# psmyth94/mamba-clip

Measured on AMD Instinct MI355X. Metric: image-text pairs/sec (whole node) + selective_scan HBM GB/s, higher is better.
Workload: dtype bf16; 1 GPU; C2: ViT-B/16 image + Mamba-130M text, contrastive train step (fwd+bwd+AdamW), amp_bf16; model=vit_b16-mamba130m, global_batch=256, per_gpu_batch=256, seq_len=77, image_size=224, input=resident, step_launch=eager, parallelism=dp1, library_gemm_selection=tunableop-file

## Files before the change

mamba-clip_amd/csrc/scan_bwd_pair.hip:

```cpp
#include "scan_common.h"

namespace mc {
namespace scan {

constexpr int kQW = 4;
constexpr int kQCh = 32;
constexpr int kQN = 16;
constexpr int kQP = 4;
constexpr int kQT = 8;
constexpr int kQSub = kS / kQT;
static_assert(kS == 32 && kQSub == 4 && kFineS == kQT, "the pair backward walks the forward's 32-position chunks "
              "in 8-position sub-tiles (the fine saved-state interval)");

struct BwdPairArgs {
  int batch, dim, seqlen, n_groups, n_states, nblk, total_blocks;
  int state_ratio;
  int64_t u_bs, u_ds, dt_bs, dt_ds, z_bs, z_ds, go_bs, go_ds;
  int64_t du_bs, du_ds, ddt_bs, ddt_ds, dz_bs, dz_ds;
  int64_t B_bs, B_gs, B_ns, C_bs, C_gs, C_ns;
  const void* u; const void* delta; const void* z; const void* dout;
  const void* B; const void* C;
  const float* A; const float* D; const float* delta_bias; const float* chunk_states;
  void* du; void* ddelta; void* dz;
  float* slab_bc;
  float* slab_a;
  float* slab_d;
  float* slab_bias;
};

template <int kCtrl>
__device__ __forceinline__ float qperm(float v) {
  return __int_as_float(__builtin_amdgcn_update_dpp(0, __float_as_int(v), kCtrl, 0xF, 0xF, true));
}
constexpr int kQpEven = 0xA0;
constexpr int kQpOdd = 0xF5;
constexpr int kQpXor1 = 0xB1;
constexpr int kQpXor2 = 0x4E;

__device__ __forceinline__ float halve_bit3(float a, float b) {
  float r;
  asm volatile("s_nop 1\n\t"
               "v_add_f32_dpp %0, %1, %1 row_ror:8 row_mask:0xf bank_mask:0x3\n\t"
               "v_add_f32_dpp %0, %2, %2 row_ror:8 row_mask:0xf bank_mask:0xc"
               : "=&v"(r) : "v"(a), "v"(b));
  return r;
}
__device__ __forceinline__ float halve_bit2(float a, float b) {
  float r;
  asm volatile("s_nop 1\n\t"
               "v_add_f32_dpp %0, %1, %1 row_shl:4 row_mask:0xf bank_mask:0x5\n\t"
               "v_add_f32_dpp %0, %2, %2 row_shr:4 row_mask:0xf bank_mask:0xa"
               : "=&v"(r) : "v"(a), "v"(b));
  return r;
}

__device__ __forceinline__ float pair_finish(f32x2 a, f32x2 b, int h) {
  float sa, sb, r;
  asm("v_add_f32_e32 %0, %1, %2" : "=v"(sa) : "v"(a.x), "v"(a.y));
  asm("v_add_f32_e32 %0, %1, %2" : "=v"(sb) : "v"(b.x), "v"(b.y));
  const float keep = h ? sb : sa, send = h ? sa : sb;
  asm("s_nop 1\n\t"
      "v_add_f32_dpp %0, %1, %2 quad_perm:[1,0,3,2] row_mask:0xf bank_mask:0xf bound_ctrl:1"
      : "=v"(r) : "v"(send), "v"(keep));
  return r;
}

__device__ __forceinline__ float pair_reduce16(f32x2 (&v)[8], int lane) {
  asm volatile("s_nop 1" : "+v"(v[0]), "+v"(v[1]), "+v"(v[2]), "+v"(v[3]), "+v"(v[4]), "+v"(v[5]), "+v"(v[6]),
               "+v"(v[7]));
#pragma unroll
  for (int t = 0; t < 4; ++t) {
    auto rx = __builtin_amdgcn_permlane32_swap(__float_as_uint(v[t].x), __float_as_uint(v[t + 4].x), false, false);
    auto ry = __builtin_amdgcn_permlane32_swap(__float_as_uint(v[t].y), __float_as_uint(v[t + 4].y), false, false);
    v[t] = f32x2{__uint_as_float(rx[0]), __uint_as_float(ry[0])} + f32x2{__uint_as_float(rx[1]), __uint_as_float(ry[1])};
  }
#pragma unroll
  for (int t = 0; t < 2; ++t) {
    auto rx = __builtin_amdgcn_permlane16_swap(__float_as_uint(v[t].x), __float_as_uint(v[t + 2].x), false, false);
    auto ry = __builtin_amdgcn_permlane16_swap(__float_as_uint(v[t].y), __float_as_uint(v[t + 2].y), false, false);
    v[t] = f32x2{__uint_as_float(rx[0]), __uint_as_float(ry[0])} + f32x2{__uint_as_float(rx[1]), __uint_as_float(ry[1])};
  }
  const float x = halve_bit3(v[0].x, v[1].x), y = halve_bit3(v[0].y, v[1].y);
  const float r = halve_bit2(x, y);
  return r + qperm<kQpXor2>(r);
}

__device__ __forceinline__ void glds16_asm(const void* gsrc, uint32_t m0v) {
  uint32_t keep;
  asm volatile("s_mov_b32 %0, m0\n\ts_mov_b32 m0, %2\n\ts_nop 0\n\tglobal_load_lds_dwordx4 %1, off\n\ts_mov_b32 m0, %0"
               : "=&s"(keep) : "v"(gsrc), "s"(m0v) : "memory");
}

template <typename TI>
__device__ __forceinline__ uint2 buf_ld8(__amdgpu_buffer_rsrc_t r, uint32_t off) {
  return __builtin_bit_cast(uint2, __builtin_amdgcn_raw_buffer_load_b64(r, off, 0, 0));
}
__device__ __forceinline__ void buf_st8(__amdgpu_buffer_rsrc_t r, uint32_t off, uint2 v) {
  typedef unsigned u32x2_t __attribute__((ext_vector_type(2)));
  __builtin_amdgcn_raw_buffer_store_b64(__builtin_bit_cast(u32x2_t, v), r, off, 0, 0);
}
template <typename TI>
__device__ __forceinline__ f32x2 elem2(uint2 w, int i) {
  const uint4 q = make_uint4(w.x, w.y, 0u, 0u);
  return f32x2{elem_f<TI>(q, 2 * i), elem_f<TI>(q, 2 * i + 1)};
}

template <typename TI, bool kSP, bool kZ, bool kFine>
__global__ __launch_bounds__(64 * kQW, 2) void scan_bwd_pair_kernel(const BwdPairArgs a) {
  using TW = TI;
  constexpr int kWV = 16 / (int)sizeof(TW);
  constexpr int kWL = 8 / kWV;
  constexpr int kDbcW = kS * 2 * kQN;
  extern __shared__ __attribute__((aligned(16))) char smem[];
  const int tid = threadIdx.x;
  const int lane = tid & 63;
  const int wave = __builtin_amdgcn_readfirstlane(tid >> 6);
  f32x4* bcq = reinterpret_cast<f32x4*>(smem) + wave * (kS * 2 * kQP);
  float* dbc_base = reinterpret_cast<float*>(smem + (size_t)kQW * kS * 2 * kQP * 16);
  f32x4* xst = reinterpret_cast<f32x4*>(dbc_base + 2 * kQW * kDbcW) + wave * ((kQSub - 1) * 2 * 64);

  const int lin = xcd_remap(blockIdx.x, a.total_blocks);
  const int wblk = lin % a.nblk;
  const int bg = lin / a.nblk;
  const int g = bg % a.n_groups, b = bg / a.n_groups;
  const int H = a.dim / a.n_groups;
  const int row0 = wblk * (kQCh * kQW) + wave * kQCh;
  const int nrows = max(0, min(kQCh, H - row0));
  const int ch = lane >> 1, h = lane & 1;
  const bool my_ok = ch < nrows;
  const int my_r = max(0, min(ch, nrows - 1));
  const int dbase = g * H + min(row0, H - 1);
  const int my_dc = dbase + my_r;
  const int L_ = a.seqlen;
  constexpr bool hasZ = kZ;

  auto rows_rsrc = [&](const void* base, int64_t bs, int64_t ds) __attribute__((always_inline)) {
    return make_rsrc(reinterpret_cast<const TI*>(base) + (int64_t)b * bs + (int64_t)dbase * ds,
                     nrows > 0 ? (uint32_t)(((int64_t)(nrows - 1) * ds + L_) * (int64_t)sizeof(TI)) : 0u);
  };
  const __amdgpu_buffer_rsrc_t rs_u = rows_rsrc(a.u, a.u_bs, a.u_ds);
  const __amdgpu_buffer_rsrc_t rs_d = rows_rsrc(a.delta, a.dt_bs, a.dt_ds);
  const __amdgpu_buffer_rsrc_t rs_z = rows_rsrc(hasZ ? a.z : a.u, hasZ ? a.z_bs : a.u_bs, hasZ ? a.z_ds : a.u_ds);
  const __amdgpu_buffer_rsrc_t rs_g = rows_rsrc(a.dout, a.go_bs, a.go_ds);
  const __amdgpu_buffer_rsrc_t rs_du = rows_rsrc(a.du, a.du_bs, a.du_ds);
  const __amdgpu_buffer_rsrc_t rs_dd = rows_rsrc(a.ddelta, a.ddt_bs, a.ddt_ds);
  const __amdgpu_buffer_rsrc_t rs_dz = rows_rsrc(hasZ ? a.dz : a.du, hasZ ? a.dz_bs : a.du_bs, hasZ ? a.dz_ds : a.du_ds);
  const uint32_t ro_u = (uint32_t)(my_r * a.u_ds), ro_d = (uint32_t)(my_r * a.dt_ds);
  const uint32_t ro_z = (uint32_t)(my_r * (hasZ ? a.z_ds : a.u_ds)), ro_g = (uint32_t)(my_r * a.go_ds);
  const uint32_t ro_du = (uint32_t)(my_r * a.du_ds), ro_dd = (uint32_t)(my_r * a.ddt_ds);
  const uint32_t ro_dz = (uint32_t)(my_r * (hasZ ? a.dz_ds : a.du_ds));
  const uint32_t st_mask = my_ok ? 0u : 0x80000000u;

  const __amdgpu_buffer_rsrc_t rs_B = make_rsrc(reinterpret_cast<const TW*>(a.B) + (int64_t)b * a.B_bs + (int64_t)g * a.B_gs,
                                                (uint32_t)((15 * a.B_ns + L_) * (int64_t)sizeof(TW)));
  const __amdgpu_buffer_rsrc_t rs_C = make_rsrc(reinterpret_cast<const TW*>(a.C) + (int64_t)b * a.C_bs + (int64_t)g * a.C_gs,
                                                (uint32_t)((15 * a.C_ns + L_) * (int64_t)sizeof(TW)));
  const uint32_t bo_B = (uint32_t)(((lane >> 2) * a.B_ns + 8 * (lane & 3)) * (int64_t)sizeof(TW));
  const uint32_t bo_C = (uint32_t)(((lane >> 2) * a.C_ns + 8 * (lane & 3)) * (int64_t)sizeof(TW));
  const uint32_t cs_rs = kFine ? (uint32_t)kQN : (uint32_t)(a.n_states * kQN);
  const uint32_t cs_ks = kFine ? (uint32_t)(a.dim * kQN) : (uint32_t)kQN;
  const __amdgpu_buffer_rsrc_t rs_cs =
      make_rsrc(a.chunk_states + (int64_t)b * a.dim * a.n_states * kQN + (int64_t)dbase * cs_rs,
                nrows > 0 ? ((uint32_t)(nrows - 1) * cs_rs + (uint32_t)(a.n_states - 1) * cs_ks + kQN) * 4u : 0u);

  f32x2 A2[kQP], hcar[kQP], dA2[kQP];
#pragma unroll
  for (int p = 0; p < kQP; ++p) {
    const float* ap = a.A + (int64_t)my_dc * kQN + 8 * h + 2 * p;
    A2[p] = f32x2{ap[0], ap[1]} * kLog2e;
    hcar[p] = f32x2{0.f, 0.f};
    dA2[p] = f32x2{0.f, 0.f};
  }
  const float Dv = a.D ? a.D[my_dc] : 0.f;
  const float biasv = a.delta_bias ? a.delta_bias[my_dc] : 0.f;
  float dDacc = 0.f, dbacc = 0.f;

  uint4 pB[kWL], pC[kWL];
  f32x4 px[2];
  auto load_chunk = [&](int c) __attribute__((always_inline)) {
    const uint32_t lo = c >= 0 ? (uint32_t)(c * kS) * (uint32_t)sizeof(TW) : 0x80000000u;
#pragma unroll
    for (int k = 0; k < kWL; ++k) {
      pB[k] = buf_ld16(rs_B, (bo_B + lo) + (uint32_t)(k * 16));
      pC[k] = buf_ld16(rs_C, (bo_C + lo) + (uint32_t)(k * 16));
    }
    const uint32_t ox = c > 0 ? ((uint32_t)my_r * cs_rs + (uint32_t)(c * (kFine ? kS / kQT : 1) - 1) * cs_ks + 8 * h) * 4u
                              : 0x80000000u;
    px[0] = __builtin_bit_cast(f32x4, buf_ld16(rs_cs, ox));
    px[1] = __builtin_bit_cast(f32x4, buf_ld16(rs_cs, ox + 16));
  };
  uint2 nu, nd, nz, ng;
  auto load_raw = [&](int pos) __attribute__((always_inline)) {
    const uint32_t e = (uint32_t)(pos + 4 * h);
    nu = buf_ld8<TI>(rs_u, (ro_u + e) * 2u);
    nd = buf_ld8<TI>(rs_d, (ro_d + e) * 2u);
    ng = buf_ld8<TI>(rs_g, (ro_g + e) * 2u);
    if constexpr (hasZ) {
      nz = buf_ld8<TI>(rs_z, (ro_z + e) * 2u);
    }
  };

  struct Sc {
    f32x2 dt[4], dtu[4], gy[4];
    f32x2 own_dt[2], own_gy[2];
  };
  auto scalars = [&](uint2 ru, uint2 rd, uint2 rz, uint2 rg, bool want_gy, Sc& sc) __attribute__((always_inline)) {
    f32x2 odt[2], odtu[2], ogy[2];
#pragma unroll
    for (int i = 0; i < 2; ++i) {
      const f32x2 r = elem2<TI>(rd, i) + biasv;
      const f32x2 dt = kSP ? softplus2_log1p(r) : r;
      odt[i] = dt;
      odtu[i] = my_ok ? dt * elem2<TI>(ru, i) : f32x2{0.f, 0.f};
      if (want_gy) {
        const f32x2 go = elem2<TI>(rg, i);
        const f32x2 gy = hasZ ? go * silu2(elem2<TI>(rz, i)) : go;
        ogy[i] = my_ok ? gy : f32x2{0.f, 0.f};
      }
    }
#pragma unroll
    for (int i = 0; i < 2; ++i) {
      sc.dt[i] = f32x2{qperm<kQpEven>(odt[i].x), qperm<kQpEven>(odt[i].y)};
      sc.dt[2 + i] = f32x2{qperm<kQpOdd>(odt[i].x), qperm<kQpOdd>(odt[i].y)};
      sc.dtu[i] = f32x2{qperm<kQpEven>(odtu[i].x), qperm<kQpEven>(odtu[i].y)};
      sc.dtu[2 + i] = f32x2{qperm<kQpOdd>(odtu[i].x), qperm<kQpOdd>(odtu[i].y)};
      if (want_gy) {
        sc.gy[i] = f32x2{qperm<kQpEven>(ogy[i].x), qperm<kQpEven>(ogy[i].y)};
        sc.gy[2 + i] = f32x2{qperm<kQpOdd>(ogy[i].x), qperm<kQpOdd>(ogy[i].y)};
        sc.own_gy[i] = ogy[i];
      }
      sc.own_dt[i] = odt[i];
    }
  };
  auto bpair = [&](int t, int p) __attribute__((always_inline)) -> f32x2 {
    return reinterpret_cast<const f32x2*>(bcq + t * (2 * kQP) + h * kQP + p)[0];
  };
  auto bquad = [&](int t, int p) __attribute__((always_inline)) -> f32x4 { return bcq[t * (2 * kQP) + h * kQP + p]; };

  const int nch = (L_ + kS - 1) / kS;
  constexpr bool fine = kFine;
  typedef __attribute__((address_space(3))) char lds_char_t;
  const uint32_t xst_lds = __builtin_amdgcn_readfirstlane((uint32_t)(uintptr_t)(lds_char_t*)(reinterpret_cast<char*>(xst)));
  const float* cs_lane = a.chunk_states + (int64_t)b * a.dim * a.n_states * kQN + (int64_t)(dbase + my_r) * kQN + 8 * h;
  auto issue_fine = [&](int c) __attribute__((always_inline)) {
#pragma unroll
    for (int s = 0; s < kQSub - 1; ++s) {
      const float* src = cs_lane + (int64_t)min(c * (kS / kQT) + s, a.n_states - 1) * cs_ks;
      glds16_asm(src, xst_lds + (uint32_t)(2 * s) * 1024u);
      glds16_asm(src + 4, xst_lds + (uint32_t)(2 * s + 1) * 1024u);
    }
  };
  if (fine) {
    issue_fine(nch - 1);
    __builtin_amdgcn_s_waitcnt(0x0F70);
  }
  load_chunk(nch - 1);
  load_raw((nch - 1) * kS + (fine ? kQT * (min(kQSub, (L_ - (nch - 1) * kS) / kQT) - 1) : 0));
  int buf = 0;
  for (int c = nch - 1; c >= 0; --c) {
    const int l0 = c * kS;
    const int nsub = min(kQSub, (L_ - l0) / kQT);
    float* dbc = dbc_base + (buf * kQW + wave) * kDbcW;

    {
      const int n = lane >> 2, q = lane & 3;
      float* dst = reinterpret_cast<float*>(bcq) + ((n >> 3) * kQP + ((n & 7) >> 1)) * 4 + (n & 1);
#pragma unroll
      for (int k = 0; k < kWL; ++k)
#pragma unroll
        for (int e = 0; e < kWV; ++e) {
          const int t = 8 * q + k * kWV + e;
          dst[t * (2 * kQP * 4)] = elem_f<TW>(pB[k], e);
          dst[t * (2 * kQP * 4) + 2] = elem_f<TW>(pC[k], e);
        }
    }
    f32x2 x0[kQP];
    x0[0] = px[0].lo; x0[1] = px[0].hi; x0[2] = px[1].lo; x0[3] = px[1].hi;
    if (!my_ok) {
#pragma unroll
      for (int p = 0; p < kQP; ++p) x0[p] = f32x2{0.f, 0.f};
    }
    if (fine) __builtin_amdgcn_s_waitcnt(0x0F70);
    load_chunk(c - 1);
    wave_lds_sync();

    if constexpr (fine) {
    } else {
      f32x2 x[kQP];
#pragma unroll
      for (int p = 0; p < kQP; ++p) x[p] = x0[p];
#pragma unroll 1
      for (int s = 0; s + 1 < nsub; ++s) {
        const uint2 ru = nu, rd = nd, rz = nz, rg = ng;
        load_raw(l0 + kQT * (s + 1));
        Sc sc;
        scalars(ru, rd, rz, rg, false, sc);
#pragma unroll
        for (int t = 0; t < kQT; ++t) {
#pragma unroll
          for (int p = 0; p < kQP; ++p) {
            const f32x2 arg = (t & 1) ? pk_mul_bcast<1>(A2[p], sc.dt[t >> 1]) : pk_mul_bcast<0>(A2[p], sc.dt[t >> 1]);
            const f32x2 aa = f32x2{fast_exp2(arg.x), fast_exp2(arg.y)};
            const f32x2 bb = bpair(kQT * s + t, p);
            const f32x2 bu = (t & 1) ? pk_mul_bcast<1>(bb, sc.dtu[t >> 1]) : pk_mul_bcast<0>(bb, sc.dtu[t >> 1]);
            x[p] = aa * x[p] + bu;
          }
        }
        xst[(2 * s) * 64 + lane] = f32x4{x[0].x, x[0].y, x[1].x, x[1].y};
        xst[(2 * s + 1) * 64 + lane] = f32x4{x[2].x, x[2].y, x[3].x, x[3].y};
      }
    }
    wave_lds_sync();

#pragma unroll 1
    for (int s = nsub - 1; s >= 0; --s) {
      const uint2 ru = nu, rd = nd, rz = nz, rg = ng;
      load_raw(s > 0 ? l0 + kQT * (s - 1) : (fine ? l0 - kQT : l0 - kS));
      Sc sc;
      scalars(ru, rd, rz, rg, true, sc);
      f32x4 xi01, xi23;
      {
        const int sl = s > 0 ? s - 1 : 0;
        const f32x4 l01 = xst[(2 * sl) * 64 + lane], l23 = xst[(2 * sl + 1) * 64 + lane];
        xi01 = s > 0 ? l01 : f32x4{x0[0].x, x0[0].y, x0[1].x, x0[1].y};
        xi23 = s > 0 ? l23 : f32x4{x0[2].x, x0[2].y, x0[3].x, x0[3].y};
      }
      f32x2 S2[kQT], Q2[kQT];
      f32x2 Y2[kQT];
#pragma unroll
      for (int t = 0; t < kQT; ++t) Y2[t] = f32x2{0.f, 0.f};
#pragma unroll
      for (int t = 0; t < kQT; ++t) S2[t] = Q2[t] = f32x2{0.f, 0.f};

#pragma unroll
      for (int p = 0; p < kQP; ++p) {
        __builtin_amdgcn_sched_barrier(0);
        f32x2 a2p = A2[p];
        asm volatile("" : "+v"(a2p));
        const f32x2 xin = p == 0 ? xi01.lo : (p == 1 ? xi01.hi : (p == 2 ? xi23.lo : xi23.hi));
        f32x2 as[kQT], xs[kQT];
#pragma unroll
        for (int t = 0; t < kQT; ++t) {
          const f32x2 arg = (t & 1) ? pk_mul_bcast<1>(a2p, sc.dt[t >> 1]) : pk_mul_bcast<0>(a2p, sc.dt[t >> 1]);
          as[t] = f32x2{fast_exp2(arg.x), fast_exp2(arg.y)};
        }
        {
          f32x2 x = xin;
#pragma unroll
          for (int t = 0; t < kQT; ++t) {
            const f32x2 bb = bpair(kQT * s + t, p);
            const f32x2 bu = (t & 1) ? pk_mul_bcast<1>(bb, sc.dtu[t >> 1]) : pk_mul_bcast<0>(bb, sc.dtu[t >> 1]);
            x = as[t] * x + bu;
            xs[t] = x;
          }
        }
        {
          f32x2 red[kQT];
#pragma unroll
          for (int t = 0; t < kQT; ++t)
            red[t] = (t & 1) ? pk_mul_bcast<1>(xs[t], sc.gy[t >> 1]) : pk_mul_bcast<0>(xs[t], sc.gy[t >> 1]);
          const float v = pair_reduce16(red, lane);
          if ((lane & 2) == 0)
            dbc[((kQT * s + (lane >> 3)) * 2 + 1) * kQN + 8 * h + 2 * p + ((lane >> 2) & 1)] = v;
        }
        __builtin_amdgcn_sched_barrier(0);
        {
          f32x2 lam, dap = dA2[p], ha;
          f32x2 red[kQT];
          f32x4 qn = bquad(kQT * s + kQT - 1, p);
#pragma unroll
          for (int t = kQT - 1; t >= 0; --t) {
            const f32x4 q = qn;
            if (t > 0) qn = bquad(kQT * s + t - 1, p);
            lam = (t & 1) ? pk_fma_bcast<1>(q.hi, sc.gy[t >> 1], t == kQT - 1 ? hcar[p] : ha)
                          : pk_fma_bcast<0>(q.hi, sc.gy[t >> 1], t == kQT - 1 ? hcar[p] : ha);
            if (hasZ) Y2[t] = q.hi * xs[t] + Y2[t];
            S2[t] = lam * q.lo + S2[t];
            red[t] = (t & 1) ? pk_mul_bcast<1>(lam, sc.dtu[t >> 1]) : pk_mul_bcast<0>(lam, sc.dtu[t >> 1]);
            ha = lam * as[t];
            const f32x2 hax = ha * (t > 0 ? xs[t - 1] : xin);
            Q2[t] = hax * a2p + Q2[t];
            dap = (t & 1) ? pk_fma_bcast<1>(hax, sc.dt[t >> 1], dap) : pk_fma_bcast<0>(hax, sc.dt[t >> 1], dap);
          }
          asm volatile("" : "+v"(ha), "+v"(dap));
#pragma unroll
          for (int t = 0; t < kQT; ++t) asm volatile("" : "+v"(S2[t]), "+v"(Q2[t]));
#pragma unroll
          for (int t = 0; t < kQT; ++t) asm volatile("" : "+v"(Y2[t]));
          hcar[p] = ha;
          dA2[p] = dap;
          const float v = pair_reduce16(red, lane);
          if ((lane & 2) == 0)
            dbc[((kQT * s + (lane >> 3)) * 2 + 0) * kQN + 8 * h + 2 * p + ((lane >> 2) & 1)] = v;
        }
      }
      __builtin_amdgcn_sched_barrier(0);

      float fS[4], fQ[4];
#pragma unroll
      for (int e = 0; e < 4; ++e) {
        fS[e] = pair_finish(S2[e], S2[4 + e], h);
        fQ[e] = pair_finish(Q2[e], Q2[4 + e], h) * kLn2;
      }
      float fY[4];
#pragma unroll
      for (int e = 0; e < 4; ++e) fY[e] = pair_finish(Y2[e], Y2[4 + e], h);
      float o_du[4], o_dd[4], o_dz[4];
#pragma unroll
      for (int i = 0; i < 2; ++i) {
        const f32x2 uu = elem2<TI>(ru, i);
        const f32x2 rr = elem2<TI>(rd, i) + biasv;
        const f32x2 dt = sc.own_dt[i], gy = sc.own_gy[i];
        const f32x2 S = f32x2{fS[2 * i], fS[2 * i + 1]}, Q = f32x2{fQ[2 * i], fQ[2 * i + 1]};
        f32x2 sg = f32x2{1.f, 1.f};
        if (kSP) {
          const f32x2 ep = f32x2{fast_exp2(-rr.x * kLog2e), fast_exp2(-rr.y * kLog2e)} + 1.f;
          sg = f32x2{rr.x > 20.f ? 1.f : fast_rcp(ep.x), rr.y > 20.f ? 1.f : fast_rcp(ep.y)};
        }
        const f32x2 du = Dv * gy + dt * S;
        const f32x2 dd = (uu * S + Q) * sg;
        o_du[2 * i] = du.x; o_du[2 * i + 1] = du.y;
        o_dd[2 * i] = dd.x; o_dd[2 * i + 1] = dd.y;
        if (hasZ) {
          const f32x2 zz = elem2<TI>(rz, i), go = elem2<TI>(rg, i);
          const f32x2 ez = f32x2{fast_exp2(-zz.x * kLog2e), fast_exp2(-zz.y * kLog2e)} + 1.f;
          const f32x2 sz = f32x2{fast_rcp(ez.x), fast_rcp(ez.y)};
          const f32x2 gz = go * sz * (1.f + zz * (1.f - sz));
          const f32x2 dz = gz * (Dv * uu + f32x2{fY[2 * i], fY[2 * i + 1]});
          o_dz[2 * i] = dz.x; o_dz[2 * i + 1] = dz.y;
        }
        if (my_ok) {
          const f32x2 gu = gy * uu;
          dDacc += gu.x + gu.y;
          dbacc += dd.x + dd.y;
        }
      }
      const uint32_t e0 = (uint32_t)(l0 + kQT * s + 4 * h);
      buf_st8(rs_du, ((ro_du + e0) * 2u) | st_mask, make_uint2(cvt_pk2<TI>(o_du[0], o_du[1]), cvt_pk2<TI>(o_du[2], o_du[3])));
      buf_st8(rs_dd, ((ro_dd + e0) * 2u) | st_mask, make_uint2(cvt_pk2<TI>(o_dd[0], o_dd[1]), cvt_pk2<TI>(o_dd[2], o_dd[3])));
      if (hasZ)
        buf_st8(rs_dz, ((ro_dz + e0) * 2u) | st_mask, make_uint2(cvt_pk2<TI>(o_dz[0], o_dz[1]), cvt_pk2<TI>(o_dz[2], o_dz[3])));
    }

    if (fine && c > 0) issue_fine(c - 1);
    lds_barrier();
    {
      float* slab = a.slab_bc + (((int64_t)bg * a.nblk + wblk) * L_ + l0) * (2 * kQN);
      const float* src = dbc_base + buf * kQW * kDbcW;
      for (int f = tid; f < kDbcW / 4; f += 64 * kQW) {
        f32x4 acc = reinterpret_cast<const f32x4*>(src)[f];
#pragma unroll
        for (int w = 1; w < kQW; ++w) acc += reinterpret_cast<const f32x4*>(src + w * kDbcW)[f];
        if (4 * f < (L_ - l0) * 2 * kQN) reinterpret_cast<f32x4*>(slab)[f] = acc;
      }
    }
    buf ^= 1;
  }

  if (my_ok) {
#pragma unroll
    for (int p = 0; p < kQP; ++p) {
      const int n0 = 8 * h + 2 * p;
      a.slab_a[((int64_t)b * kQN + n0) * a.dim + my_dc] = dA2[p].x;
      a.slab_a[((int64_t)b * kQN + n0 + 1) * a.dim + my_dc] = dA2[p].y;
    }
  }
  const float dD2 = dDacc + qperm<kQpXor1>(dDacc), db2 = dbacc + qperm<kQpXor1>(dbacc);
  if (my_ok && h == 0) {
    a.slab_d[(int64_t)b * a.dim + my_dc] = dD2;
    a.slab_bias[(int64_t)b * a.dim + my_dc] = db2;
  }
}

size_t bwd_pair_lds_bytes() {
  return (size_t)kQW * kS * 2 * kQP * 16 + (size_t)2 * kQW * kS * 2 * kQN * 4 + (size_t)kQW * (kQSub - 1) * 2 * 64 * 16;
}
int bwd_pair_nblk(int H) { return (H + kQCh * kQW - 1) / (kQCh * kQW); }

bool bwd_pair_ok(const mc_scan_bwd_params* p) {
  const int ib = p->itype == MC_DTYPE_F32 ? 4 : 2;
  const int wb = p->wtype == MC_DTYPE_F32 ? 4 : 2;
  if (ib != 2 || p->wtype != p->itype || p->dstate != kQN || p->seqlen % 8 || p->reverse_groups || p->u_groups)
    return false;
  auto rows = [&](const void* t, int64_t bs, int64_t ds) {
    return !t || (aligned16(t) && bs % 8 == 0 && ds % 8 == 0 &&
                  ((int64_t)(kQCh * kQW - 1) * (ds < 0 ? -ds : ds) + p->seqlen) * 2 < ((int64_t)1 << 31));
  };
  auto bc = [&](const void* t, int64_t bs, int64_t gs, int64_t ns) {
    const int64_t v = 16 / wb;
    return aligned16(t) && bs % v == 0 && gs % v == 0 && ns % v == 0 && ns >= 0 &&
           (15 * ns + p->seqlen) * wb < ((int64_t)1 << 31);
  };
  return rows(p->u, p->u_batch_stride, p->u_dim_stride) &&
         rows(p->delta, p->delta_batch_stride, p->delta_dim_stride) &&
         rows(p->z, p->z_batch_stride, p->z_dim_stride) && rows(p->dout, p->dout_batch_stride, p->dout_dim_stride) &&
         rows(p->du, p->du_batch_stride, p->du_dim_stride) &&
         rows(p->ddelta, p->ddelta_batch_stride, p->ddelta_dim_stride) &&
         rows(p->dz, p->dz_batch_stride, p->dz_dim_stride) &&
         bc(p->B, p->B_batch_stride, p->B_group_stride, p->B_dstate_stride) &&
         bc(p->C, p->C_batch_stride, p->C_group_stride, p->C_dstate_stride) &&
         (int64_t)kQCh * kQW * mc_scan_n_states(p->seqlen, p->state_interval) * kQN * 4 < ((int64_t)1 << 31);
}

template <typename TI>
static void launch_pair_t(const BwdPairArgs& a, bool sp, bool zy, hipStream_t s) {
  const size_t lds = bwd_pair_lds_bytes();
  const dim3 grid(a.total_blocks), block(64 * kQW);
  if (a.state_ratio != 1) {
    if (sp && zy) hipLaunchKernelGGL((scan_bwd_pair_kernel<TI, true, true, true>), grid, block, lds, s, a);
    else if (sp) hipLaunchKernelGGL((scan_bwd_pair_kernel<TI, true, false, true>), grid, block, lds, s, a);
    else if (zy) hipLaunchKernelGGL((scan_bwd_pair_kernel<TI, false, true, true>), grid, block, lds, s, a);
    else hipLaunchKernelGGL((scan_bwd_pair_kernel<TI, false, false, true>), grid, block, lds, s, a);
    return;
  }
  if (sp && zy) hipLaunchKernelGGL((scan_bwd_pair_kernel<TI, true, true, false>), grid, block, lds, s, a);
  else if (sp) hipLaunchKernelGGL((scan_bwd_pair_kernel<TI, true, false, false>), grid, block, lds, s, a);
  else if (zy) hipLaunchKernelGGL((scan_bwd_pair_kernel<TI, false, true, false>), grid, block, lds, s, a);
  else hipLaunchKernelGGL((scan_bwd_pair_kernel<TI, false, false, false>), grid, block, lds, s, a);
}

void launch_bwd_pair(const mc_scan_bwd_params* p, float* slab_bc, float* slab_a, float* slab_d, float* slab_bias,
                     int nblk, hipStream_t s) {
  BwdPairArgs a;
  a.batch = p->batch; a.dim = p->dim; a.seqlen = p->seqlen; a.n_groups = p->n_groups;
  a.n_states = mc_scan_n_states(p->seqlen, p->state_interval);
  a.state_ratio = p->state_interval == kFineS ? kS / kFineS : 1;
  a.nblk = nblk;
  a.total_blocks = p->batch * p->n_groups * nblk;
  a.u_bs = p->u_batch_stride; a.u_ds = p->u_dim_stride;
  a.dt_bs = p->delta_batch_stride; a.dt_ds = p->delta_dim_stride;
  a.z_bs = p->z_batch_stride; a.z_ds = p->z_dim_stride;
  a.go_bs = p->dout_batch_stride; a.go_ds = p->dout_dim_stride;
  a.du_bs = p->du_batch_stride; a.du_ds = p->du_dim_stride;
  a.ddt_bs = p->ddelta_batch_stride; a.ddt_ds = p->ddelta_dim_stride;
  a.dz_bs = p->dz_batch_stride; a.dz_ds = p->dz_dim_stride;
  a.B_bs = p->B_batch_stride; a.B_gs = p->B_group_stride; a.B_ns = p->B_dstate_stride;
  a.C_bs = p->C_batch_stride; a.C_gs = p->C_group_stride; a.C_ns = p->C_dstate_stride;
  a.u = p->u; a.delta = p->delta; a.z = p->z; a.dout = p->dout; a.B = p->B; a.C = p->C;
  a.A = p->A; a.D = p->D; a.delta_bias = p->delta_bias; a.chunk_states = p->chunk_states;
  a.du = p->du; a.ddelta = p->ddelta; a.dz = p->dz;
  a.slab_bc = slab_bc; a.slab_a = slab_a; a.slab_d = slab_d; a.slab_bias = slab_bias;
  const bool sp = p->delta_softplus != 0, zy = p->z != nullptr;
  if (p->itype == MC_DTYPE_BF16) launch_pair_t<bf16_t>(a, sp, zy, s);
  else launch_pair_t<f16_t>(a, sp, zy, s);
}

}
}
```

mamba-clip_amd/csrc/scan_common.h:

```cpp
#pragma once

#include "mc_common.h"
#include "../../include/mc_scan.h"

namespace mc {
namespace scan {

constexpr int kT = 32;
constexpr int kS = MC_SCAN_CHUNK;
constexpr int kFineS = MC_SCAN_STATE_INTERVAL_FINE;
constexpr int kRows = 64;

inline int padded_dstate(int dstate) { return dstate <= 8 ? 8 : (dstate <= 16 ? 16 : 32); }

static_assert(kRows == 64, "wave_lds_sync() is only valid for one-wave workgroups");
__device__ __forceinline__ void wave_lds_sync() { asm volatile("" ::: "memory"); }

__device__ __forceinline__ void lds_barrier() {
  asm volatile("" ::: "memory");
  __builtin_amdgcn_s_waitcnt(0xC07F);
  __builtin_amdgcn_s_barrier();
  asm volatile("" ::: "memory");
}

__device__ __forceinline__ int opaque_lane_id() {
  int v;
  asm volatile("v_mbcnt_lo_u32_b32 %0, -1, 0\n\tv_mbcnt_hi_u32_b32 %0, -1, %0" : "=v"(v));
  return v;
}

__device__ __forceinline__ f32x2 softplus2_log1p(f32x2 x) {
  const f32x2 arg = x * kLog2e;
  const f32x2 t = f32x2{fast_exp2(-fabsf(arg.x)), fast_exp2(-fabsf(arg.y))};
  const f32x2 tp = t + 1.f;
  const f32x2 lg = f32x2{fast_log2(tp.x), fast_log2(tp.y)};
  return lg * kLn2 + f32x2{fmaxf(x.x, 0.f), fmaxf(x.y, 0.f)};
}
__device__ __forceinline__ f32x2 silu2(f32x2 z) {
  const f32x2 arg = z * -kLog2e;
  const f32x2 ep = f32x2{fast_exp2(arg.x), fast_exp2(arg.y)} + 1.f;
  return z * f32x2{fast_rcp(ep.x), fast_rcp(ep.y)};
}

template <int kHi>
__device__ __forceinline__ f32x2 pk_mul_bcast(f32x2 a, f32x2 s) {
  if constexpr (kHi) {
    float x, y;
    asm("v_mul_f32 %0, %2, %4\n\tv_mul_f32 %1, %3, %4" : "=&v"(x), "=&v"(y) : "v"(a.x), "v"(a.y), "v"(s.y));
    return f32x2{x, y};
  } else {
    f32x2 r;
    asm("v_pk_mul_f32 %0, %1, %2 op_sel_hi:[1,0]" : "=v"(r) : "v"(a), "v"(s));
    return r;
  }
}
template <int kHi>
__device__ __forceinline__ f32x2 pk_fma_bcast(f32x2 a, f32x2 s, f32x2 c) {
  if constexpr (kHi) {
    float x, y;
    asm("v_fma_f32 %0, %2, %4, %5\n\tv_fma_f32 %1, %3, %4, %6" : "=&v"(x), "=&v"(y)
        : "v"(a.x), "v"(a.y), "v"(s.y), "v"(c.x), "v"(c.y));
    return f32x2{x, y};
  } else {
    f32x2 r;
    asm("v_pk_fma_f32 %0, %1, %2, %3 op_sel_hi:[1,0,1]" : "=v"(r) : "v"(a), "v"(s), "v"(c));
    return r;
  }
}
__device__ __forceinline__ f32x2 hi_to_lo(f32x2 s) {
  f32x2 r = __builtin_nondeterministic_value(r);
  r.x = s.y;
  return r;
}

struct FwdArgs {
  int batch, dim, seqlen, dstate, n_groups, n_chunks, n_states, nblk, total_blocks;
  int softplus;
  int64_t u_bs, u_ds, dt_bs, dt_ds, z_bs, z_ds, o_bs, o_ds;
  const void* u; const void* delta; const float* A; const float* bct;
  const float* D; const void* z; const float* delta_bias;
  void* out; float* chunk_states; float* last_state;
  void* out_y; int64_t y_bs, y_ds;
  int rev_groups, u_groups;
  const void* B; const void* C;
  int64_t B_bs, B_gs, B_ns, C_bs, C_gs, C_ns;
  int state_interval;
};

int validate_common(int batch, int dim, int seqlen, int dstate, int n_groups, int itype, int wtype, const char* who);
bool vec_ok(const void* p, int64_t s0, int64_t s1, int64_t s2, int elem_bytes);

}
}
```

Measured before the change: 3769 image-text pairs/sec.

## Stage scan backward row inputs through LDS with async global-to-LDS loads

```diff
diff --git a/mamba-clip_amd/csrc/scan_bwd_pair.hip b/mamba-clip_amd/csrc/scan_bwd_pair.hip
--- a/mamba-clip_amd/csrc/scan_bwd_pair.hip
+++ b/mamba-clip_amd/csrc/scan_bwd_pair.hip
@@ -91,10 +91,6 @@
                : "=&s"(keep) : "v"(gsrc), "s"(m0v) : "memory");
 }
 
-template <typename TI>
-__device__ __forceinline__ uint2 buf_ld8(__amdgpu_buffer_rsrc_t r, uint32_t off) {
-  return __builtin_bit_cast(uint2, __builtin_amdgcn_raw_buffer_load_b64(r, off, 0, 0));
-}
 __device__ __forceinline__ void buf_st8(__amdgpu_buffer_rsrc_t r, uint32_t off, uint2 v) {
   typedef unsigned u32x2_t __attribute__((ext_vector_type(2)));
   __builtin_amdgcn_raw_buffer_store_b64(__builtin_bit_cast(u32x2_t, v), r, off, 0, 0);
@@ -115,9 +111,13 @@
   const int tid = threadIdx.x;
   const int lane = tid & 63;
   const int wave = __builtin_amdgcn_readfirstlane(tid >> 6);
-  f32x4* bcq = reinterpret_cast<f32x4*>(smem) + wave * (kS * 2 * kQP);
-  float* dbc_base = reinterpret_cast<float*>(smem + (size_t)kQW * kS * 2 * kQP * 16);
-  f32x4* xst = reinterpret_cast<f32x4*>(dbc_base + 2 * kQW * kDbcW) + wave * ((kQSub - 1) * 2 * 64);
+  static_assert(sizeof(TI) == 2 && kWV == 8 && kWL == 1, "16-bit rows: 8 positions per 16-B piece");
+  constexpr int kBcqQ = kS * 2 * kQP;
+  f32x4* bcq_base = reinterpret_cast<f32x4*>(smem);
+  float* dbc_base = reinterpret_cast<float*>(smem + (size_t)2 * kBcqQ * 16);
+  f32x4* xst = reinterpret_cast<f32x4*>(dbc_base + kQW * kDbcW) + wave * ((kQSub - 1) * 2 * 64);
+  const char* stg = smem + (size_t)2 * kBcqQ * 16 + (size_t)kQW * kDbcW * 4 + (size_t)kQW * (kQSub - 1) * 2 * 64 * 16 +
+                    (size_t)wave * (4 * kStageArrayBytes);
 
   const int lin = xcd_remap(blockIdx.x, a.total_blocks);
   const int wblk = lin % a.nblk;
@@ -138,15 +138,16 @@
     return make_rsrc(reinterpret_cast<const TI*>(base) + (int64_t)b * bs + (int64_t)dbase * ds,
                      nrows > 0 ? (uint32_t)(((int64_t)(nrows - 1) * ds + L_) * (int64_t)sizeof(TI)) : 0u);
   };
-  const __amdgpu_buffer_rsrc_t rs_u = rows_rsrc(a.u, a.u_bs, a.u_ds);
-  const __amdgpu_buffer_rsrc_t rs_d = rows_rsrc(a.delta, a.dt_bs, a.dt_ds);
-  const __amdgpu_buffer_rsrc_t rs_z = rows_rsrc(hasZ ? a.z : a.u, hasZ ? a.z_bs : a.u_bs, hasZ ? a.z_ds : a.u_ds);
-  const __amdgpu_buffer_rsrc_t rs_g = rows_rsrc(a.dout, a.go_bs, a.go_ds);
+  auto rows_ptr = [&](const void* base, int64_t bs, int64_t ds) __attribute__((always_inline)) {
+    return reinterpret_cast<const TI*>(base) + (int64_t)b * bs + (int64_t)dbase * ds;
+  };
+  const TI* gb_u = rows_ptr(a.u, a.u_bs, a.u_ds);
+  const TI* gb_d = rows_ptr(a.delta, a.dt_bs, a.dt_ds);
+  const TI* gb_g = rows_ptr(a.dout, a.go_bs, a.go_ds);
+  const TI* gb_z = hasZ ? rows_ptr(a.z, a.z_bs, a.z_ds) : gb_u;
   const __amdgpu_buffer_rsrc_t rs_du = rows_rsrc(a.du, a.du_bs, a.du_ds);
   const __amdgpu_buffer_rsrc_t rs_dd = rows_rsrc(a.ddelta, a.ddt_bs, a.ddt_ds);
   const __amdgpu_buffer_rsrc_t rs_dz = rows_rsrc(hasZ ? a.dz : a.du, hasZ ? a.dz_bs : a.du_bs, hasZ ? a.dz_ds : a.du_ds);
-  const uint32_t ro_u = (uint32_t)(my_r * a.u_ds), ro_d = (uint32_t)(my_r * a.dt_ds);
-  const uint32_t ro_z = (uint32_t)(my_r * (hasZ ? a.z_ds : a.u_ds)), ro_g = (uint32_t)(my_r * a.go_ds);
   const uint32_t ro_du = (uint32_t)(my_r * a.du_ds), ro_dd = (uint32_t)(my_r * a.ddt_ds);
   const uint32_t ro_dz = (uint32_t)(my_r * (hasZ ? a.dz_ds : a.du_ds));
   const uint32_t st_mask = my_ok ? 0u : 0x80000000u;
@@ -155,8 +156,9 @@
                                                 (uint32_t)((15 * a.B_ns + L_) * (int64_t)sizeof(TW)));
   const __amdgpu_buffer_rsrc_t rs_C = make_rsrc(reinterpret_cast<const TW*>(a.C) + (int64_t)b * a.C_bs + (int64_t)g * a.C_gs,
                                                 (uint32_t)((15 * a.C_ns + L_) * (int64_t)sizeof(TW)));
-  const uint32_t bo_B = (uint32_t)(((lane >> 2) * a.B_ns + 8 * (lane & 3)) * (int64_t)sizeof(TW));
-  const uint32_t bo_C = (uint32_t)(((lane >> 2) * a.C_ns + 8 * (lane & 3)) * (int64_t)sizeof(TW));
+  const int bc_t0 = 8 * wave + 2 * (lane & 3);
+  const uint32_t bo_B = (uint32_t)(((lane >> 2) * a.B_ns + bc_t0) * (int64_t)sizeof(TW));
+  const uint32_t bo_C = (uint32_t)(((lane >> 2) * a.C_ns + bc_t0) * (int64_t)sizeof(TW));
   const uint32_t cs_rs = kFine ? (uint32_t)kQN : (uint32_t)(a.n_states * kQN);
   const uint32_t cs_ks = kFine ? (uint32_t)(a.dim * kQN) : (uint32_t)kQN;
   const __amdgpu_buffer_rsrc_t rs_cs =
@@ -175,29 +177,35 @@
   const float biasv = a.delta_bias ? a.delta_bias[my_dc] : 0.f;
   float dDacc = 0.f, dbacc = 0.f;
 
-  uint4 pB[kWL], pC[kWL];
+  uint32_t pB, pC;
   f32x4 px[2];
   auto load_chunk = [&](int c) __attribute__((always_inline)) {
     const uint32_t lo = c >= 0 ? (uint32_t)(c * kS) * (uint32_t)sizeof(TW) : 0x80000000u;
-#pragma unroll
-    for (int k = 0; k < kWL; ++k) {
-      pB[k] = buf_ld16(rs_B, (bo_B + lo) + (uint32_t)(k * 16));
-      pC[k] = buf_ld16(rs_C, (bo_C + lo) + (uint32_t)(k * 16));
-    }
+    pB = __builtin_amdgcn_raw_buffer_load_b32(rs_B, bo_B + lo, 0, 0);
+    pC = __builtin_amdgcn_raw_buffer_load_b32(rs_C, bo_C + lo, 0, 0);
     const uint32_t ox = c > 0 ? ((uint32_t)my_r * cs_rs + (uint32_t)(c * (kFine ? kS / kQT : 1) - 1) * cs_ks + 8 * h) * 4u
                               : 0x80000000u;
     px[0] = __builtin_bit_cast(f32x4, buf_ld16(rs_cs, ox));
     px[1] = __builtin_bit_cast(f32x4, buf_ld16(rs_cs, ox + 16));
   };
-  uint2 nu, nd, nz, ng;
-  auto load_raw = [&](int pos) __attribute__((always_inline)) {
-    const uint32_t e = (uint32_t)(pos + 4 * h);
-    nu = buf_ld8<TI>(rs_u, (ro_u + e) * 2u);
-    nd = buf_ld8<TI>(rs_d, (ro_d + e) * 2u);
-    ng = buf_ld8<TI>(rs_g, (ro_g + e) * 2u);
-    if constexpr (hasZ) {
-      nz = buf_ld8<TI>(rs_z, (ro_z + e) * 2u);
-    }
+  auto store_bc = [&](int c) __attribute__((always_inline)) {
+    const int n = lane >> 2;
+    float* dst = reinterpret_cast<float*>(bcq_base + (c & 1) * kBcqQ) + bc_t0 * (2 * kQP * 4) +
+                 ((n >> 3) * kQP + ((n & 7) >> 1)) * 4 + (n & 1);
+    const uint4 wB = make_uint4(pB, 0u, 0u, 0u), wC = make_uint4(pC, 0u, 0u, 0u);
+#pragma unroll
+    for (int e = 0; e < 2; ++e) {
+      dst[e * (2 * kQP * 4)] = elem_f<TW>(wB, e);
+      dst[e * (2 * kQP * 4) + 2] = elem_f<TW>(wC, e);
+    }
+  };
+  const char* stg_lane = stg + stage_row_byte(ch, 4 * h);
+  auto read_rows = [&](int s, uint2& ru, uint2& rd, uint2& rz, uint2& rg) __attribute__((always_inline)) {
+    const char* p = stg_lane + s * (kQT * 2);
+    ru = *reinterpret_cast<const uint2*>(p);
+    rd = *reinterpret_cast<const uint2*>(p + kStageArrayBytes);
+    rg = *reinterpret_cast<const uint2*>(p + 2 * kStageArrayBytes);
+    rz = hasZ ? *reinterpret_cast<const uint2*>(p + 3 * kStageArrayBytes) : make_uint2(0u, 0u);
   };
 
   struct Sc {
@@ -232,6 +240,7 @@
       sc.own_dt[i] = odt[i];
     }
   };
+  const f32x4* bcq = bcq_base;
   auto bpair = [&](int t, int p) __attribute__((always_inline)) -> f32x2 {
     return reinterpret_cast<const f32x2*>(bcq + t * (2 * kQP) + h * kQP + p)[0];
   };
@@ -250,37 +259,38 @@
       glds16_asm(src + 4, xst_lds + (uint32_t)(2 * s + 1) * 1024u);
     }
   };
-  if (fine) {
-    issue_fine(nch - 1);
-    __builtin_amdgcn_s_waitcnt(0x0F70);
-  }
+  const uint32_t stg_lds = __builtin_amdgcn_readfirstlane((uint32_t)(uintptr_t)(lds_char_t*)(const_cast<char*>(stg)));
+  auto issue_rows = [&](int c) __attribute__((always_inline)) {
+    const int ol = opaque_lane_id();
+    auto one = [&](const TI* gb, int64_t ds, int arr) __attribute__((always_inline)) {
+#pragma unroll
+      for (int i = 0; i < 2; ++i)
+        glds16_asm(gb + stage_src_elem(ol, i, c, nrows, L_, ds),
+                   stg_lds + (uint32_t)(arr * kStageArrayBytes) + stage_dst_byte(0, i));
+    };
+    one(gb_u, a.u_ds, 0);
+    one(gb_d, a.dt_ds, 1);
+    one(gb_g, a.go_ds, 2);
+    if constexpr (hasZ) one(gb_z, a.z_ds, 3);
+  };
+  issue_rows(nch - 1);
+  if (fine) issue_fine(nch - 1);
   load_chunk(nch - 1);
-  load_raw((nch - 1) * kS + (fine ? kQT * (min(kQSub, (L_ - (nch - 1) * kS) / kQT) - 1) : 0));
-  int buf = 0;
+  store_bc(nch - 1);
+  lds_barrier();
+  float* dbc = dbc_base + wave * kDbcW;
   for (int c = nch - 1; c >= 0; --c) {
     const int l0 = c * kS;
     const int nsub = min(kQSub, (L_ - l0) / kQT);
-    float* dbc = dbc_base + (buf * kQW + wave) * kDbcW;
-
-    {
-      const int n = lane >> 2, q = lane & 3;
-      float* dst = reinterpret_cast<float*>(bcq) + ((n >> 3) * kQP + ((n & 7) >> 1)) * 4 + (n & 1);
-#pragma unroll
-      for (int k = 0; k < kWL; ++k)
-#pragma unroll
-        for (int e = 0; e < kWV; ++e) {
-          const int t = 8 * q + k * kWV + e;
-          dst[t * (2 * kQP * 4)] = elem_f<TW>(pB[k], e);
-          dst[t * (2 * kQP * 4) + 2] = elem_f<TW>(pC[k], e);
-        }
-    }
+    bcq = bcq_base + (c & 1) * kBcqQ;
+
     f32x2 x0[kQP];
     x0[0] = px[0].lo; x0[1] = px[0].hi; x0[2] = px[1].lo; x0[3] = px[1].hi;
     if (!my_ok) {
 #pragma unroll
       for (int p = 0; p < kQP; ++p) x0[p] = f32x2{0.f, 0.f};
     }
-    if (fine) __builtin_amdgcn_s_waitcnt(0x0F70);
+    __builtin_amdgcn_s_waitcnt(0x0F70);
     load_chunk(c - 1);
     wave_lds_sync();
 
@@ -291,8 +301,8 @@
       for (int p = 0; p < kQP; ++p) x[p] = x0[p];
 #pragma unroll 1
       for (int s = 0; s + 1 < nsub; ++s) {
-        const uint2 ru = nu, rd = nd, rz = nz, rg = ng;
-        load_raw(l0 + kQT * (s + 1));
+        uint2 ru, rd, rz, rg;
+        read_rows(s, ru, rd, rz, rg);
         Sc sc;
         scalars(ru, rd, rz, rg, false, sc);
 #pragma unroll
@@ -310,12 +320,16 @@
         xst[(2 * s + 1) * 64 + lane] = f32x4{x[2].x, x[2].y, x[3].x, x[3].y};
       }
     }
-    wave_lds_sync();
+    lds_barrier();
 
 #pragma unroll 1
     for (int s = nsub - 1; s >= 0; --s) {
-      const uint2 ru = nu, rd = nd, rz = nz, rg = ng;
-      load_raw(s > 0 ? l0 + kQT * (s - 1) : (fine ? l0 - kQT : l0 - kS));
+      uint2 ru, rd, rz, rg;
+      read_rows(s, ru, rd, rz, rg);
+      if (s == 0 && c > 0) {
+        asm volatile("s_waitcnt lgkmcnt(0)" ::: "memory");
+        issue_rows(c - 1);
+      }
       Sc sc;
       scalars(ru, rd, rz, rg, true, sc);
       f32x4 xi01, xi23;
@@ -442,11 +456,12 @@
         buf_st8(rs_dz, ((ro_dz + e0) * 2u) | st_mask, make_uint2(cvt_pk2<TI>(o_dz[0], o_dz[1]), cvt_pk2<TI>(o_dz[2], o_dz[3])));
     }
 
+    if (c > 0) store_bc(c - 1);
     if (fine && c > 0) issue_fine(c - 1);
     lds_barrier();
     {
       float* slab = a.slab_bc + (((int64_t)bg * a.nblk + wblk) * L_ + l0) * (2 * kQN);
-      const float* src = dbc_base + buf * kQW * kDbcW;
+      const float* src = dbc_base;
       for (int f = tid; f < kDbcW / 4; f += 64 * kQW) {
         f32x4 acc = reinterpret_cast<const f32x4*>(src)[f];
 #pragma unroll
@@ -454,7 +469,6 @@
         if (4 * f < (L_ - l0) * 2 * kQN) reinterpret_cast<f32x4*>(slab)[f] = acc;
       }
     }
-    buf ^= 1;
   }
 
   if (my_ok) {
@@ -473,8 +487,11 @@
 }
 
 size_t bwd_pair_lds_bytes() {
-  return (size_t)kQW * kS * 2 * kQP * 16 + (size_t)2 * kQW * kS * 2 * kQN * 4 + (size_t)kQW * (kQSub - 1) * 2 * 64 * 16;
-}
+  return (size_t)2 * kS * 2 * kQP * 16 + (size_t)kQW * kS * 2 * kQN * 4 + (size_t)kQW * (kQSub - 1) * 2 * 64 * 16 +
+         (size_t)kQW * 4 * kStageArrayBytes;
+}
+static_assert(2 * (2 * kS * 2 * kQP * 16 + kQW * kS * 2 * kQN * 4 + kQW * (kQSub - 1) * 2 * 64 * 16 + kQW * 4 * kStageArrayBytes) <=
+              160 * 1024, "two workgroups per CU");
 int bwd_pair_nblk(int H) { return (H + kQCh * kQW - 1) / (kQCh * kQW); }
 
 bool bwd_pair_ok(const mc_scan_bwd_params* p) {
diff --git a/mamba-clip_amd/csrc/scan_common.h b/mamba-clip_amd/csrc/scan_common.h
--- a/mamba-clip_amd/csrc/scan_common.h
+++ b/mamba-clip_amd/csrc/scan_common.h
@@ -73,6 +73,17 @@
   return r;
 }
 
+constexpr int kStageRowBytes = kS * 2;
+constexpr int kStageInstrBytes = 64 * 16;
+constexpr int kStageArrayBytes = 32 * kStageRowBytes;
+__host__ __device__ inline int64_t stage_src_elem(int lane, int i, int chunk, int nrows, int seqlen, int64_t row_stride) {
+  const int last_row = nrows > 0 ? nrows - 1 : 0;
+  const int row = 16 * i + (lane >> 2), pos = chunk * kS + 8 * (lane & 3);
+  return (int64_t)(row < last_row ? row : last_row) * row_stride + (pos < seqlen - 8 ? pos : seqlen - 8);
+}
+__host__ __device__ inline uint32_t stage_row_byte(int row, int pos) { return (uint32_t)(row * kStageRowBytes + pos * 2); }
+__host__ __device__ inline uint32_t stage_dst_byte(int lane, int i) { return (uint32_t)(i * kStageInstrBytes + lane * 16); }
+
 struct FwdArgs {
   int batch, dim, seqlen, dstate, n_groups, n_chunks, n_states, nblk, total_blocks;
   int softplus;
```

After: 3844 image-text pairs/sec (median of 6 runs). +2.0%, better.
